# xuelunshen/gim

Hardware: AMD Instinct MI355X
Metric: image-pairs/sec at 640x480 (higher is better)
Workload: dtype fp16

## Files before the change

gim_amd/csrc/bneck_tail.hip:

```cpp
#include "gim_common.h"

namespace {

template <int P, int N1, int NW = 8, bool DS = false> struct Cfg {
    static constexpr int ROWS = 32 * NW;
    static constexpr int LDS_LIMIT = (NW == 8 ? 160 : 80) * 1024;
    static constexpr int C4 = 4 * P;
    static constexpr int KD = DS ? 2 * P : 0;
    static constexpr int CH = (P == 128 && !DS) ? 64 : 32;
    static constexpr int NCHUNK = C4 / CH;
    static constexpr int W3ROW = (P + KD) * 2;
    static constexpr int W3C = CH * W3ROW;
    static constexpr int W1ROW = CH * 2;
    static constexpr int W1C = N1 * W1ROW;
    static constexpr int BUF = W3C + W1C;
    static constexpr int PROW = CH * 2;
    static constexpr int PATCH = 32 * PROW;
    static constexpr int NBUF = (3 * BUF + NW * PATCH + (C4 + N1) * 4 <= LDS_LIMIT) ? 3 : 2;
    static constexpr int OFF_PATCH = NBUF * BUF;
    static constexpr int OFF_BIAS = OFF_PATCH + NW * PATCH;
    static constexpr int SMEM = OFF_BIAS + (C4 + N1) * 4;
    static constexpr int PIECES = BUF / 1024;
    static constexpr int PPW = PIECES / NW;
    static constexpr int IPC = PATCH / 1024;
    static_assert(SMEM <= LDS_LIMIT && PIECES % NW == 0 && (P == 128 || P == 256) && (NW == 8 || NW == 4) && NW * 4096 <= NBUF * BUF && (!DS || P == 128) &&
                  W3C % 1024 == 0, "LDS map");
};

struct Args {
    const unsigned short* t2;
    const unsigned short* res;
    unsigned short* xo;
    unsigned short* t1n;
    const unsigned short* w3;
    const unsigned short* w1n;
    const float* b3;
    const float* b1n;
    int M;
    int act1;
    unsigned w3_bytes, w1n_bytes;
    int* health;
    const unsigned short* xin;
    int Ho, Wo, Hin, Win;
};

typedef __attribute__((address_space(3))) void lds_t;
GIM_TT_DECL(bneck_tail)

typedef gim_u32x4_t u32x4_t;
__device__ __forceinline__ void dma16(const u32x4_t rsrc, unsigned lds_addr, unsigned voff) { gim_dma16(rsrc, lds_addr, voff); }
__device__ __forceinline__ u32x4_t make_rsrc(const void* p, unsigned bytes) { return gim_make_rsrc(p, bytes); }
template <int N> __device__ __forceinline__ void tail_wait() { asm volatile("s_waitcnt vmcnt(%0)" : : "n"(N) : "memory"); }

template <int ROWB> __device__ __forceinline__ int swz(int row, int slot) {
    if constexpr (ROWB >= 256) return (slot & ~15) | ((slot & 15) ^ (row & 15));
    else if constexpr (ROWB == 128) return slot ^ ((row >> 1) & 7);
    else return slot ^ ((row >> 2) & 3);
}
template <int PROW> __device__ __forceinline__ int pswz(int px, int slot) {
    if constexpr (PROW == 128) return slot ^ (px & 7);
    else return slot ^ ((px >> 2) & 3);
}

template <int P, int N1, int NW, bool DS>
__device__ __forceinline__ void issue_chunk(const u32x4_t rw3, const u32x4_t rw1, unsigned smem_addr, int buf, int q, int w, int lane) {
    typedef Cfg<P, N1, NW, DS> C;
    constexpr int S3 = C::W3ROW / 16, S1 = C::W1ROW / 16;
    const unsigned base = smem_addr + (unsigned)(buf * C::BUF);
#pragma unroll
    for (int k = 0; k < C::PPW; ++k) {
        const int pc = w + NW * k;
        if (pc < C::W3C / 1024) {
            const int idx = pc * 64 + lane, n = idx / S3, d = idx % S3;
            const unsigned voff = (unsigned)((q * C::CH + n) * C::W3ROW + (swz<C::W3ROW>(n, d) << 4));
            dma16(rw3, base + (unsigned)(pc * 1024), voff);
        } else {
            const int p1 = pc - C::W3C / 1024;
            const int idx = p1 * 64 + lane, n = idx / S1, d = idx % S1;
            const unsigned voff = (unsigned)((q * N1 + n) * C::W1ROW + (swz<C::W1ROW>(n, d) << 4));
            dma16(rw1, base + (unsigned)(C::W3C + p1 * 1024), voff);
        }
    }
}

template <int P, int N1, int NW, bool DS = false>
__global__ void __launch_bounds__(NW * 64, 2) bneck_tail_kernel(const Args a) {
    typedef Cfg<P, N1, NW, DS> C;
    constexpr int ROWS = C::ROWS;
    constexpr int C4 = C::C4, CH = C::CH, NCHUNK = C::NCHUNK, PROW = C::PROW;
    constexpr int NF = N1 / 32;
    constexpr int TF = CH / 32;
    constexpr int LPP = PROW / 16;
    constexpr int PPI = 64 / LPP;
    extern __shared__ __attribute__((aligned(16))) char smem[];
    const int lane = threadIdx.x & 63, l31 = lane & 31, lh = lane >> 5;
    const int w = __builtin_amdgcn_readfirstlane(threadIdx.x >> 6);
    bool hbig = false;
    const size_t prow0 = (size_t)blockIdx.x * ROWS + w * 32;
    char* patch = smem + C::OFF_PATCH + w * C::PATCH;

    GIM_TT(bneck_tail, w, 0);
    unsigned long long tt_wait = 0, tt_c3 = 0, tt_epi = 0, tt_c1 = 0, tt_a = 0, tt_b = 0;
    (void)tt_wait; (void)tt_c3; (void)tt_epi; (void)tt_c1; (void)tt_a; (void)tt_b;
    const u32x4_t rw3 = make_rsrc(a.w3, a.w3_bytes), rw1 = make_rsrc(a.w1n, a.w1n_bytes);
    const unsigned smem_addr = __builtin_amdgcn_readfirstlane((unsigned)(size_t)(lds_t*)smem);
    issue_chunk<P, N1, NW, DS>(rw3, rw1, smem_addr, 0, 0, w, lane);
    float* bias = (float*)(smem + C::OFF_BIAS);
    for (int t = threadIdx.x; t < (C4 + N1) / 4; t += NW * 64) {
        if (t < C4 / 4) *(float4*)(bias + 4 * t) = *(const float4*)(a.b3 + 4 * t);
        else *(float4*)(bias + 4 * t) = *(const float4*)(a.b1n + 4 * t - C4);
    }
    bf16x8_t t2[P / 16];
    {
        const unsigned short* tp = a.t2 + (prow0 + l31) * P + 8 * lh;
#pragma unroll
        for (int s = 0; s < P / 16; ++s) t2[s] = *(const bf16x8_t*)(tp + 16 * s);
    }
#pragma unroll
    for (int s = 0; s < P / 16; ++s) asm volatile("" : "+v"(t2[s]));
    bf16x8_t xi[DS ? C::KD / 16 : 1];
    if constexpr (DS) {
        const size_t m = prow0 + l31;
        const int ox = (int)(m % (size_t)a.Wo);
        const size_t r_ = m / (size_t)a.Wo;
        const int oy = (int)(r_ % (size_t)a.Ho);
        const size_t ib = r_ / (size_t)a.Ho;
        const unsigned short* xp = a.xin + ((ib * a.Hin + 2 * oy) * a.Win + 2 * ox) * C::KD + 8 * lh;
#pragma unroll
        for (int s = 0; s < C::KD / 16; ++s) xi[s] = *(const bf16x8_t*)(xp + 16 * s);
#pragma unroll
        for (int s = 0; s < C::KD / 16; ++s) asm volatile("" : "+v"(xi[s]));
    }
    const u32x4_t rres = make_rsrc(DS ? (const void*)a.t2 : (const void*)a.res, DS ? 16u : (unsigned)((size_t)a.M * C4 * 2));
    const unsigned patch_addr = smem_addr + (unsigned)(C::OFF_PATCH + w * C::PATCH);
    const int ipx = lane / LPP, isl = lane % LPP;
    const unsigned id_voff = (unsigned)((prow0 + ipx) * (C4 * 2)) + (unsigned)(pswz<PROW>(ipx, isl) << 4);
    auto issue_identity = [&](const int q) __attribute__((always_inline)) {
        if constexpr (!DS) {
#pragma unroll
            for (int k = 0; k < C::IPC; ++k) dma16(rres, patch_addr + (unsigned)(k * 1024), id_voff + (unsigned)(k * PPI * C4 * 2 + q * CH * 2));
        }
    };
    issue_identity(0);
    if constexpr (C::NBUF == 3) issue_chunk<P, N1, NW, DS>(rw3, rw1, smem_addr, 1, 1, w, lane);
    __syncthreads();

    GIM_TT(bneck_tail, w, 1);
    f32x16_t c1[NF];
#pragma unroll
    for (int f = 0; f < NF; ++f) {
#pragma unroll
        for (int rg = 0; rg < 4; ++rg) {
            const float4 bb = *(const float4*)(bias + C4 + 32 * f + 8 * rg + 4 * lh);
            c1[f][rg * 4] = bb.x; c1[f][rg * 4 + 1] = bb.y; c1[f][rg * 4 + 2] = bb.z; c1[f][rg * 4 + 3] = bb.w;
        }
    }

#pragma unroll 1
    for (int q = 0; q < NCHUNK; ++q) {
        tt_a = GIM_TT_NOW();
        const bool dma_ahead = C::NBUF == 3 && q + 1 < NCHUNK;
        const bool stores_behind = q > 0 && a.xo != nullptr;
        if (dma_ahead) { if (stores_behind) tail_wait<C::PPW + C::IPC>(); else tail_wait<C::PPW>(); }
        else { if (stores_behind) tail_wait<C::IPC>(); else tail_wait<0>(); }
        __syncthreads();
        const char* wb3 = smem + (q % C::NBUF) * C::BUF;
        const char* wb1 = wb3 + C::W3C;
        tt_b = GIM_TT_NOW(); tt_wait += tt_b - tt_a;

        f32x16_t c3[TF];
#pragma unroll
        for (int f = 0; f < TF; ++f) {
#pragma unroll
            for (int rg = 0; rg < 4; ++rg) {
                const float4 bb = *(const float4*)(bias + q * CH + 32 * f + 8 * rg + 4 * lh);
                c3[f][rg * 4] = bb.x; c3[f][rg * 4 + 1] = bb.y; c3[f][rg * 4 + 2] = bb.z; c3[f][rg * 4 + 3] = bb.w;
            }
        }
#pragma unroll
        for (int s = 0; s < P / 16; ++s) {
#pragma unroll
            for (int f = 0; f < TF; ++f) {
                const int n = 32 * f + l31;
                const bf16x8_t wv = *(const bf16x8_t*)(wb3 + n * C::W3ROW + (swz<C::W3ROW>(n, 2 * s + lh) << 4));
                c3[f] = mfma_h16_32x32x16(wv, t2[s], c3[f]);
            }
        }
        if constexpr (DS) {
#pragma unroll
            for (int s = 0; s < C::KD / 16; ++s) {
#pragma unroll
                for (int f = 0; f < TF; ++f) {
                    const int n = 32 * f + l31;
                    const bf16x8_t wv = *(const bf16x8_t*)(wb3 + n * C::W3ROW + (swz<C::W3ROW>(n, 2 * (P / 16 + s) + lh) << 4));
                    c3[f] = mfma_h16_32x32x16(wv, xi[s], c3[f]);
                }
            }
        }
        tt_a = GIM_TT_NOW(); tt_c3 += tt_a - tt_b;
#pragma unroll
        for (int f = 0; f < TF; ++f) {
#pragma unroll
            for (int rg = 0; rg < 4; ++rg) {
                if constexpr (DS) {
#pragma unroll
                    for (int e = 0; e < 4; ++e) c3[f][rg * 4 + e] = fmaxf(c3[f][rg * 4 + e], 0.f);
                } else {
                    const uint2 r = *(const uint2*)(patch + l31 * PROW + (pswz<PROW>(l31, 4 * f + rg) << 4) + lh * 8);
                    c3[f][rg * 4] = fmaxf(c3[f][rg * 4] + h16_lo(r.x), 0.f);
                    c3[f][rg * 4 + 1] = fmaxf(c3[f][rg * 4 + 1] + h16_hi(r.x), 0.f);
                    c3[f][rg * 4 + 2] = fmaxf(c3[f][rg * 4 + 2] + h16_lo(r.y), 0.f);
                    c3[f][rg * 4 + 3] = fmaxf(c3[f][rg * 4 + 3] + h16_hi(r.y), 0.f);
                }
            }
        }
        asm volatile("s_waitcnt lgkmcnt(0)" ::: "memory");
        bf16x8_t xq[2 * TF];
#pragma unroll
        for (int f = 0; f < TF; ++f) {
            unsigned u[8];
#pragma unroll
            for (int rg = 0; rg < 4; ++rg) {
                u[2 * rg] = cvt_pk_h16(c3[f][rg * 4], c3[f][rg * 4 + 1]);
                u[2 * rg + 1] = cvt_pk_h16(c3[f][rg * 4 + 2], c3[f][rg * 4 + 3]);
                *(uint2*)(patch + l31 * PROW + (pswz<PROW>(l31, 4 * f + rg) << 4) + lh * 8) = make_uint2(u[2 * rg], u[2 * rg + 1]);
            }
            xq[2 * f] = __builtin_bit_cast(bf16x8_t, make_uint4(u[0], u[1], u[2], u[3]));
            xq[2 * f + 1] = __builtin_bit_cast(bf16x8_t, make_uint4(u[4], u[5], u[6], u[7]));
        }
        asm volatile("s_waitcnt lgkmcnt(0)" ::: "memory");
        const char* prd = patch + ipx * PROW + (pswz<PROW>(ipx, isl) << 4);
        uint4 x0 = *(const uint4*)(prd), x1 = *(const uint4*)(prd + PPI * PROW), x2 = x0, x3 = x0;
        if constexpr (C::IPC == 4) { x2 = *(const uint4*)(prd + 2 * PPI * PROW); x3 = *(const uint4*)(prd + 3 * PPI * PROW); }
        asm volatile("s_waitcnt lgkmcnt(0)" ::: "memory");
        h16_range_track(hbig, x0); h16_range_track(hbig, x1);
        if constexpr (C::IPC == 4) { h16_range_track(hbig, x2); h16_range_track(hbig, x3); }
        if (q + 1 < NCHUNK) issue_identity(q + 1);
        if (q + C::NBUF - 1 < NCHUNK) issue_chunk<P, N1, NW, DS>(rw3, rw1, smem_addr, (q + C::NBUF - 1) % C::NBUF, q + C::NBUF - 1, w, lane);
        if (a.xo != nullptr) {
            unsigned short* xp = a.xo + (prow0 + ipx) * C4 + CH * q + isl * 8;
            *(uint4*)(xp) = x0; *(uint4*)(xp + (size_t)PPI * C4) = x1;
            if constexpr (C::IPC == 4) { *(uint4*)(xp + (size_t)2 * PPI * C4) = x2; *(uint4*)(xp + (size_t)3 * PPI * C4) = x3; }
        }
        tt_b = GIM_TT_NOW(); tt_epi += tt_b - tt_a;
#pragma unroll
        for (int s = 0; s < 2 * TF; ++s) {
#pragma unroll
            for (int f = 0; f < NF; ++f) {
                const int n = 32 * f + l31;
                const bf16x8_t wv = *(const bf16x8_t*)(wb1 + n * C::W1ROW + (swz<C::W1ROW>(n, 2 * s + lh) << 4));
                c1[f] = mfma_h16_32x32x16(wv, xq[s], c1[f]);
            }
        }
        tt_a = GIM_TT_NOW(); tt_c1 += tt_a - tt_b;
    }
    GIM_TT(bneck_tail, w, 2);
    GIM_TT_SET(bneck_tail, w, 4, tt_wait); GIM_TT_SET(bneck_tail, w, 5, tt_c3); GIM_TT_SET(bneck_tail, w, 6, tt_epi); GIM_TT_SET(bneck_tail, w, 7, tt_c1);
    __syncthreads();
    char* opatch = smem + w * 4096;
    const bool relu1 = a.act1 == GIM_ACT_RELU;
#pragma unroll
    for (int h2 = 0; h2 < NF / 2; ++h2) {
#pragma unroll
        for (int ff = 0; ff < 2; ++ff)
#pragma unroll
            for (int rg = 0; rg < 4; ++rg) {
                const f32x16_t& c = c1[2 * h2 + ff];
                const float lo = relu1 ? 0.f : -INFINITY;
                *(uint2*)(opatch + l31 * 128 + (((4 * ff + rg) ^ (l31 & 7)) << 4) + lh * 8) =
                    make_uint2(cvt_pk_h16(fmaxf(c[rg * 4], lo), fmaxf(c[rg * 4 + 1], lo)), cvt_pk_h16(fmaxf(c[rg * 4 + 2], lo), fmaxf(c[rg * 4 + 3], lo)));
            }
        asm volatile("s_waitcnt lgkmcnt(0)" ::: "memory");
#pragma unroll
        for (int it = 0; it < 4; ++it) {
            const int px = it * 8 + (lane >> 3), sl = lane & 7;
            const uint4 v = *(const uint4*)(opatch + px * 128 + ((sl ^ (px & 7)) << 4));
            *(uint4*)(a.t1n + (prow0 + px) * N1 + 64 * h2 + sl * 8) = v;
        }
        asm volatile("s_waitcnt lgkmcnt(0)" ::: "memory");
    }
    h16_range_flag(a.health, hbig);
    GIM_TT(bneck_tail, w, 3);
}

template <int P, int N1, int NW = 8, bool DS = false>
int launch_tail(const Args& a, hipStream_t s) {
    typedef Cfg<P, N1, NW, DS> C;
    static GimPerDevice attr;
    if (attr.needed()) {
        hipError_t e = hipFuncSetAttribute((const void*)bneck_tail_kernel<P, N1, NW, DS>, hipFuncAttributeMaxDynamicSharedMemorySize, C::SMEM);
        if (e != hipSuccess) { gim_set_error("bneck_tail: hipFuncSetAttribute(%d B LDS): %s", C::SMEM, hipGetErrorString(e)); return GIM_ERR_LAUNCH; }
        attr.done();
    }
    hipLaunchKernelGGL((bneck_tail_kernel<P, N1, NW, DS>), dim3((unsigned)(a.M / C::ROWS)), dim3(NW * 64), C::SMEM, s, a);
    return gim_check_launch("bneck_tail");
}

int tail_entry(int P, const void* t2, const void* res, void* x_out, void* t1_next, const void* w3, const void* w1n,
               const float* b3, const float* b1n, int M, int n_next, int act_next, int32_t* health, gim_stream_t stream) {
    GIM_REQUIRE(t2 && res && t1_next && w3 && w1n && b3 && b1n, "bneck_tail: NULL pointer");
    GIM_REQUIRE(act_next == GIM_ACT_RELU || act_next == GIM_ACT_NONE, "bneck_tail: activation of the next conv1 must be relu or none");
    GIM_REQUIRE(M > 0 && M % 256 == 0, "bneck_tail: the pixel row count must be a multiple of 256 (got %d)", M);
    GIM_REQUIRE((int64_t)M * 4 * P * 2 < (int64_t)0xFFFFFFF0ll, "bneck_tail: tensor too large for 32-bit buffer offsets");
    Args a;
    a.t2 = (const unsigned short*)t2; a.res = (const unsigned short*)res; a.xo = (unsigned short*)x_out; a.t1n = (unsigned short*)t1_next;
    a.w3 = (const unsigned short*)w3; a.w1n = (const unsigned short*)w1n; a.b3 = b3; a.b1n = b1n; a.M = M; a.act1 = act_next;
    a.w3_bytes = (unsigned)(4 * P * P * 2); a.w1n_bytes = (unsigned)(n_next * 4 * P * 2); a.health = (int*)health;
    a.xin = nullptr; a.Ho = a.Wo = a.Hin = a.Win = 0;
    if (P == 128) {
        GIM_REQUIRE(n_next == 128 || n_next == 256, "bneck_tail128: n_next must be 128 or 256 (got %d)", n_next);
        return n_next == 128 ? launch_tail<128, 128>(a, (hipStream_t)stream) : launch_tail<128, 256>(a, (hipStream_t)stream);
    }
    GIM_REQUIRE(n_next == 256, "bneck_tail256: n_next must be 256 (got %d)", n_next);
    if (M / 256 > 256 && M / 256 < 3 * 256) return launch_tail<256, 256, 4>(a, (hipStream_t)stream);
    return launch_tail<256, 256>(a, (hipStream_t)stream);
}

}

extern "C" int GIM_FN(gim_bneck_tail128)(const void* t2, const void* res, void* x_out, void* t1_next, const void* w3, const void* w1n,
                                         const float* b3, const float* b1n, int M, int n_next, int act_next, int32_t* health, gim_stream_t stream) {
    GIM_REQUIRE(x_out, "bneck_tail128: NULL x_out");
    return tail_entry(128, t2, res, x_out, t1_next, w3, w1n, b3, b1n, M, n_next, act_next, health, stream);
}

extern "C" int GIM_FN(gim_bneck_tail128_ds)(const void* t2, const void* x_in, void* x_out, void* t1_next, const void* w3ds, const void* w1n,
                                            const float* b3ds, const float* b1n, int B, int Ho, int Wo, int Hin, int Win, int n_next, int act_next,
                                            int32_t* health, gim_stream_t stream) {
    GIM_REQUIRE(t2 && x_in && x_out && t1_next && w3ds && w1n && b3ds && b1n, "bneck_tail128_ds: NULL pointer");
    GIM_REQUIRE(act_next == GIM_ACT_RELU || act_next == GIM_ACT_NONE, "bneck_tail128_ds: activation of the next conv1 must be relu or none");
    GIM_REQUIRE(B > 0 && Ho > 0 && Wo > 0 && Hin >= 2 * Ho - 1 && Win >= 2 * Wo - 1, "bneck_tail128_ds: the input map must cover the stride-2 samples (%d x %d -> %d x %d)", Hin, Win, Ho, Wo);
    const int64_t M = (int64_t)B * Ho * Wo;
    GIM_REQUIRE(M % 256 == 0, "bneck_tail128_ds: the pixel row count must be a multiple of 256 (got %lld)", (long long)M);
    GIM_REQUIRE(M * 512 * 2 < (int64_t)0xFFFFFFF0ll, "bneck_tail128_ds: tensor too large for 32-bit buffer offsets");
    GIM_REQUIRE(n_next == 128, "bneck_tail128_ds: n_next must be 128 (got %d)", n_next);
    Args a;
    a.t2 = (const unsigned short*)t2; a.res = nullptr; a.xo = (unsigned short*)x_out; a.t1n = (unsigned short*)t1_next;
    a.w3 = (const unsigned short*)w3ds; a.w1n = (const unsigned short*)w1n; a.b3 = b3ds; a.b1n = b1n; a.M = (int)M; a.act1 = act_next;
    a.w3_bytes = (unsigned)(512 * 384 * 2); a.w1n_bytes = (unsigned)(n_next * 512 * 2); a.health = (int*)health;
    a.xin = (const unsigned short*)x_in; a.Ho = Ho; a.Wo = Wo; a.Hin = Hin; a.Win = Win;
    return launch_tail<128, 128, 8, true>(a, (hipStream_t)stream);
}

extern "C" int GIM_FN(gim_bneck_tail256)(const void* t2, const void* res, void* x_out, void* t1_next, const void* w3, const void* w1n,
                                         const float* b3, const float* b1n, int M, int n_next, int act_next, int32_t* health, gim_stream_t stream) {
    return tail_entry(256, t2, res, x_out, t1_next, w3, w1n, b3, b1n, M, n_next, act_next, health, stream);
}
```

Baseline: 816.5.

## Make bottleneck tail kernel persistent with cross-tile weight and operand prefetch

Turns the bottleneck tail kernel into a persistent kernel. The grid is capped at the CU count (two blocks per CU for 4-wave blocks), and each workgroup walks a contiguous range of row tiles. Weight chunks, identity patches and the next tile's t2/x operands are prefetched across tile boundaries, so the DMA pipeline and global loads stay busy between tiles instead of draining at every block. The x output stores now go through buffer stores, and the t1 output staging reuses a weight buffer. In exchange the wait counting and sync logic get more complex, and there are fewer workgroups to hide latency.

```diff
diff --git a/gim_amd/csrc/bneck_tail.hip b/gim_amd/csrc/bneck_tail.hip
--- a/gim_amd/csrc/bneck_tail.hip
+++ b/gim_amd/csrc/bneck_tail.hip
@@ -23,7 +23,7 @@
     static constexpr int PIECES = BUF / 1024;
     static constexpr int PPW = PIECES / NW;
     static constexpr int IPC = PATCH / 1024;
-    static_assert(SMEM <= LDS_LIMIT && PIECES % NW == 0 && (P == 128 || P == 256) && (NW == 8 || NW == 4) && NW * 4096 <= NBUF * BUF && (!DS || P == 128) &&
+    static_assert(SMEM <= LDS_LIMIT && PIECES % NW == 0 && (P == 128 || P == 256) && (NW == 8 || NW == 4) && NW * 4096 <= BUF && (!DS || P == 128) &&
                   W3C % 1024 == 0, "LDS map");
 };
 
@@ -83,7 +83,17 @@
     }
 }
 
-template <int P, int N1, int NW, bool DS = false>
+template <int A, int B, int T> __device__ __forceinline__ void tail_wait_behind(const bool dma_ahead, const bool stores_behind, const bool t1_behind) {
+    if (dma_ahead) {
+        if (stores_behind) { if (t1_behind) tail_wait<A + B + T>(); else tail_wait<A + B>(); }
+        else { if (t1_behind) tail_wait<A + T>(); else tail_wait<A>(); }
+    } else {
+        if (stores_behind) { if (t1_behind) tail_wait<B + T>(); else tail_wait<B>(); }
+        else { if (t1_behind) tail_wait<T>(); else tail_wait<0>(); }
+    }
+}
+
+template <int P, int N1, int NW = 8, bool DS = false>
 __global__ void __launch_bounds__(NW * 64, 2) bneck_tail_kernel(const Args a) {
     typedef Cfg<P, N1, NW, DS> C;
     constexpr int ROWS = C::ROWS;
@@ -92,17 +102,23 @@
     constexpr int TF = CH / 32;
     constexpr int LPP = PROW / 16;
     constexpr int PPI = 64 / LPP;
+    constexpr int T1S = NF / 2 * 4;
     extern __shared__ __attribute__((aligned(16))) char smem[];
-    const int lane = threadIdx.x & 63, l31 = lane & 31, lh = lane >> 5;
+    const int lane_id = threadIdx.x & 63, lane = lane_id, l31 = lane & 31, lh = lane >> 5;
     const int w = __builtin_amdgcn_readfirstlane(threadIdx.x >> 6);
     bool hbig = false;
-    const size_t prow0 = (size_t)blockIdx.x * ROWS + w * 32;
     char* patch = smem + C::OFF_PATCH + w * C::PATCH;
+    const int ntiles = a.M / ROWS, nwg = (int)gridDim.x, bid = (int)blockIdx.x;
+    const int tq = ntiles / nwg, tr = ntiles % nwg;
+    const int tile0 = bid * tq + (bid < tr ? bid : tr), ntile = tq + (bid < tr ? 1 : 0);
+    const int last_g = ntile * NCHUNK - 1;
+    auto prow_of = [&](const int tile) __attribute__((always_inline)) { return (size_t)tile * ROWS + w * 32; };
 
     GIM_TT(bneck_tail, w, 0);
-    unsigned long long tt_wait = 0, tt_c3 = 0, tt_epi = 0, tt_c1 = 0, tt_a = 0, tt_b = 0;
-    (void)tt_wait; (void)tt_c3; (void)tt_epi; (void)tt_c1; (void)tt_a; (void)tt_b;
+    unsigned long long tt_wait = 0, tt_c3 = 0, tt_epi = 0, tt_c1 = 0, tt_out = 0, tt_a = 0, tt_b = 0;
+    (void)tt_wait; (void)tt_c3; (void)tt_epi; (void)tt_c1; (void)tt_out; (void)tt_a; (void)tt_b;
     const u32x4_t rw3 = make_rsrc(a.w3, a.w3_bytes), rw1 = make_rsrc(a.w1n, a.w1n_bytes);
+    const __amdgpu_buffer_rsrc_t rxo = __builtin_amdgcn_make_buffer_rsrc(a.xo, (short)0, a.xo != nullptr ? (int)((unsigned)a.M * (unsigned)(C4 * 2)) : 0, 0x00020000);
     const unsigned smem_addr = __builtin_amdgcn_readfirstlane((unsigned)(size_t)(lds_t*)smem);
     issue_chunk<P, N1, NW, DS>(rw3, rw1, smem_addr, 0, 0, w, lane);
     float* bias = (float*)(smem + C::OFF_BIAS);
@@ -111,60 +127,62 @@
         else *(float4*)(bias + 4 * t) = *(const float4*)(a.b1n + 4 * t - C4);
     }
     bf16x8_t t2[P / 16];
-    {
-        const unsigned short* tp = a.t2 + (prow0 + l31) * P + 8 * lh;
+    bf16x8_t xi[DS ? C::KD / 16 : 1];
+    auto load_operands = [&](const int tile) __attribute__((always_inline)) {
+        const size_t prow = prow_of(tile);
+        const unsigned short* tp = a.t2 + (prow + l31) * P + 8 * lh;
 #pragma unroll
         for (int s = 0; s < P / 16; ++s) t2[s] = *(const bf16x8_t*)(tp + 16 * s);
-    }
-#pragma unroll
-    for (int s = 0; s < P / 16; ++s) asm volatile("" : "+v"(t2[s]));
-    bf16x8_t xi[DS ? C::KD / 16 : 1];
-    if constexpr (DS) {
-        const size_t m = prow0 + l31;
-        const int ox = (int)(m % (size_t)a.Wo);
-        const size_t r_ = m / (size_t)a.Wo;
-        const int oy = (int)(r_ % (size_t)a.Ho);
-        const size_t ib = r_ / (size_t)a.Ho;
-        const unsigned short* xp = a.xin + ((ib * a.Hin + 2 * oy) * a.Win + 2 * ox) * C::KD + 8 * lh;
-#pragma unroll
-        for (int s = 0; s < C::KD / 16; ++s) xi[s] = *(const bf16x8_t*)(xp + 16 * s);
-#pragma unroll
-        for (int s = 0; s < C::KD / 16; ++s) asm volatile("" : "+v"(xi[s]));
-    }
+        if constexpr (DS) {
+            const size_t m = prow + l31;
+            const int ox = (int)(m % (size_t)a.Wo);
+            const size_t r_ = m / (size_t)a.Wo;
+            const int oy = (int)(r_ % (size_t)a.Ho);
+            const size_t ib = r_ / (size_t)a.Ho;
+            const unsigned short* xp = a.xin + ((ib * a.Hin + 2 * oy) * a.Win + 2 * ox) * C::KD + 8 * lh;
+#pragma unroll
+            for (int s = 0; s < C::KD / 16; ++s) xi[s] = *(const bf16x8_t*)(xp + 16 * s);
+        }
+    };
+    auto fence_operands = [&]() __attribute__((always_inline)) {
+#pragma unroll
+        for (int s = 0; s < P / 16; ++s) asm volatile("" : "+v"(t2[s]));
+        if constexpr (DS) {
+#pragma unroll
+            for (int s = 0; s < C::KD / 16; ++s) asm volatile("" : "+v"(xi[s]));
+        }
+    };
+    load_operands(tile0);
     const u32x4_t rres = make_rsrc(DS ? (const void*)a.t2 : (const void*)a.res, DS ? 16u : (unsigned)((size_t)a.M * C4 * 2));
     const unsigned patch_addr = smem_addr + (unsigned)(C::OFF_PATCH + w * C::PATCH);
     const int ipx = lane / LPP, isl = lane % LPP;
-    const unsigned id_voff = (unsigned)((prow0 + ipx) * (C4 * 2)) + (unsigned)(pswz<PROW>(ipx, isl) << 4);
-    auto issue_identity = [&](const int q) __attribute__((always_inline)) {
+    const unsigned id_key = (unsigned)(ipx * (C4 * 2)) + (unsigned)(pswz<PROW>(ipx, isl) << 4);
+    auto issue_identity = [&](const int tile, const int q) __attribute__((always_inline)) {
         if constexpr (!DS) {
+            const unsigned id_voff = (unsigned)(prow_of(tile) * (C4 * 2)) + id_key;
 #pragma unroll
             for (int k = 0; k < C::IPC; ++k) dma16(rres, patch_addr + (unsigned)(k * 1024), id_voff + (unsigned)(k * PPI * C4 * 2 + q * CH * 2));
         }
     };
-    issue_identity(0);
+    issue_identity(tile0, 0);
     if constexpr (C::NBUF == 3) issue_chunk<P, N1, NW, DS>(rw3, rw1, smem_addr, 1, 1, w, lane);
+    fence_operands();
     __syncthreads();
 
     GIM_TT(bneck_tail, w, 1);
     f32x16_t c1[NF];
-#pragma unroll
-    for (int f = 0; f < NF; ++f) {
-#pragma unroll
-        for (int rg = 0; rg < 4; ++rg) {
-            const float4 bb = *(const float4*)(bias + C4 + 32 * f + 8 * rg + 4 * lh);
-            c1[f][rg * 4] = bb.x; c1[f][rg * 4 + 1] = bb.y; c1[f][rg * 4 + 2] = bb.z; c1[f][rg * 4 + 3] = bb.w;
-        }
-    }
-
-#pragma unroll 1
-    for (int q = 0; q < NCHUNK; ++q) {
+
+    auto chunk = [&](const int it, const int q, auto last_of_tile) __attribute__((always_inline)) {
+        constexpr bool LAST = decltype(last_of_tile)::value;
+        const int tile = tile0 + it, g = it * NCHUNK + q;
+        const size_t prow0 = prow_of(tile);
+        int lane = lane_id;
+        asm volatile("" : "+v"(lane));
+        const int l31 = lane & 31, lh = lane >> 5, ipx = lane / LPP, isl = lane % LPP;
         tt_a = GIM_TT_NOW();
-        const bool dma_ahead = C::NBUF == 3 && q + 1 < NCHUNK;
-        const bool stores_behind = q > 0 && a.xo != nullptr;
-        if (dma_ahead) { if (stores_behind) tail_wait<C::PPW + C::IPC>(); else tail_wait<C::PPW>(); }
-        else { if (stores_behind) tail_wait<C::IPC>(); else tail_wait<0>(); }
+        tail_wait_behind<C::PPW, C::IPC, T1S>(C::NBUF == 3 && g + 1 <= last_g, g > 0, !LAST && q == 0 && g > 0);
         __syncthreads();
-        const char* wb3 = smem + (q % C::NBUF) * C::BUF;
+        const char* wb3 = smem + (g % C::NBUF) * C::BUF;
         const char* wb1 = wb3 + C::W3C;
         tt_b = GIM_TT_NOW(); tt_wait += tt_b - tt_a;
 
@@ -196,6 +214,10 @@
                     c3[f] = mfma_h16_32x32x16(wv, xi[s], c3[f]);
                 }
             }
+        }
+        if constexpr (LAST) {
+            __builtin_amdgcn_sched_barrier(0);
+            if (it + 1 < ntile) load_operands(tile + 1);
         }
         tt_a = GIM_TT_NOW(); tt_c3 += tt_a - tt_b;
 #pragma unroll
@@ -235,12 +257,18 @@
         asm volatile("s_waitcnt lgkmcnt(0)" ::: "memory");
         h16_range_track(hbig, x0); h16_range_track(hbig, x1);
         if constexpr (C::IPC == 4) { h16_range_track(hbig, x2); h16_range_track(hbig, x3); }
-        if (q + 1 < NCHUNK) issue_identity(q + 1);
-        if (q + C::NBUF - 1 < NCHUNK) issue_chunk<P, N1, NW, DS>(rw3, rw1, smem_addr, (q + C::NBUF - 1) % C::NBUF, q + C::NBUF - 1, w, lane);
-        if (a.xo != nullptr) {
-            unsigned short* xp = a.xo + (prow0 + ipx) * C4 + CH * q + isl * 8;
-            *(uint4*)(xp) = x0; *(uint4*)(xp + (size_t)PPI * C4) = x1;
-            if constexpr (C::IPC == 4) { *(uint4*)(xp + (size_t)2 * PPI * C4) = x2; *(uint4*)(xp + (size_t)3 * PPI * C4) = x3; }
+        if (g + 1 <= last_g) { if constexpr (LAST) issue_identity(tile + 1, 0); else issue_identity(tile, q + 1); }
+        if (g + C::NBUF - 1 <= last_g) {
+            const int gn = g + C::NBUF - 1;
+            issue_chunk<P, N1, NW, DS>(rw3, rw1, smem_addr, gn % C::NBUF, gn % NCHUNK, w, lane);
+        }
+        {
+            const unsigned xv = (unsigned)(((prow0 + ipx) * C4 + CH * q + isl * 8) * 2);
+            auto st = [&](const uint4 v, const int k) __attribute__((always_inline)) {
+                __builtin_amdgcn_raw_buffer_store_b128(u32x4_t{v.x, v.y, v.z, v.w}, rxo, (int)(xv + (unsigned)(k * PPI * C4 * 2)), 0, 0);
+            };
+            st(x0, 0); st(x1, 1);
+            if constexpr (C::IPC == 4) { st(x2, 2); st(x3, 3); }
         }
         tt_b = GIM_TT_NOW(); tt_epi += tt_b - tt_a;
 #pragma unroll
@@ -253,34 +281,64 @@
             }
         }
         tt_a = GIM_TT_NOW(); tt_c1 += tt_a - tt_b;
-    }
-    GIM_TT(bneck_tail, w, 2);
+    };
+
+#pragma unroll 1
+    for (int it = 0; it < ntile; ++it) {
+#pragma unroll
+        for (int f = 0; f < NF; ++f) {
+#pragma unroll
+            for (int rg = 0; rg < 4; ++rg) {
+                const float4 bb = *(const float4*)(bias + C4 + 32 * f + 8 * rg + 4 * lh);
+                c1[f][rg * 4] = bb.x; c1[f][rg * 4 + 1] = bb.y; c1[f][rg * 4 + 2] = bb.z; c1[f][rg * 4 + 3] = bb.w;
+            }
+        }
+#pragma unroll 1
+        for (int q = 0; q < NCHUNK - 1; ++q) chunk(it, q, std::false_type());
+        chunk(it, NCHUNK - 1, std::true_type());
+        if (it + 1 == ntile) GIM_TT(bneck_tail, w, 2);
+        __syncthreads();
+        const size_t prow0 = prow_of(tile0 + it);
+        char* opatch = smem + ((it * NCHUNK + NCHUNK - 1) % C::NBUF) * C::BUF + w * 4096;
+        const bool relu1 = a.act1 == GIM_ACT_RELU;
+#pragma unroll
+        for (int h2 = 0; h2 < NF / 2; ++h2) {
+#pragma unroll
+            for (int ff = 0; ff < 2; ++ff)
+#pragma unroll
+                for (int rg = 0; rg < 4; ++rg) {
+                    const f32x16_t& c = c1[2 * h2 + ff];
+                    const float lo = relu1 ? 0.f : -INFINITY;
+                    *(uint2*)(opatch + l31 * 128 + (((4 * ff + rg) ^ (l31 & 7)) << 4) + lh * 8) =
+                        make_uint2(cvt_pk_h16(fmaxf(c[rg * 4], lo), fmaxf(c[rg * 4 + 1], lo)), cvt_pk_h16(fmaxf(c[rg * 4 + 2], lo), fmaxf(c[rg * 4 + 3], lo)));
+                }
+            asm volatile("s_waitcnt lgkmcnt(0)" ::: "memory");
+#pragma unroll
+            for (int k = 0; k < 4; ++k) {
+                const int px = k * 8 + (lane >> 3), sl = lane & 7;
+                const uint4 v = *(const uint4*)(opatch + px * 128 + ((sl ^ (px & 7)) << 4));
+                *(uint4*)(a.t1n + (prow0 + px) * N1 + 64 * h2 + sl * 8) = v;
+            }
+            asm volatile("s_waitcnt lgkmcnt(0)" ::: "memory");
+        }
+        fence_operands();
+        tt_b = GIM_TT_NOW(); tt_out += tt_b - tt_a;
+    }
     GIM_TT_SET(bneck_tail, w, 4, tt_wait); GIM_TT_SET(bneck_tail, w, 5, tt_c3); GIM_TT_SET(bneck_tail, w, 6, tt_epi); GIM_TT_SET(bneck_tail, w, 7, tt_c1);
-    __syncthreads();
-    char* opatch = smem + w * 4096;
-    const bool relu1 = a.act1 == GIM_ACT_RELU;
-#pragma unroll
-    for (int h2 = 0; h2 < NF / 2; ++h2) {
-#pragma unroll
-        for (int ff = 0; ff < 2; ++ff)
-#pragma unroll
-            for (int rg = 0; rg < 4; ++rg) {
-                const f32x16_t& c = c1[2 * h2 + ff];
-                const float lo = relu1 ? 0.f : -INFINITY;
-                *(uint2*)(opatch + l31 * 128 + (((4 * ff + rg) ^ (l31 & 7)) << 4) + lh * 8) =
-                    make_uint2(cvt_pk_h16(fmaxf(c[rg * 4], lo), fmaxf(c[rg * 4 + 1], lo)), cvt_pk_h16(fmaxf(c[rg * 4 + 2], lo), fmaxf(c[rg * 4 + 3], lo)));
-            }
-        asm volatile("s_waitcnt lgkmcnt(0)" ::: "memory");
-#pragma unroll
-        for (int it = 0; it < 4; ++it) {
-            const int px = it * 8 + (lane >> 3), sl = lane & 7;
-            const uint4 v = *(const uint4*)(opatch + px * 128 + ((sl ^ (px & 7)) << 4));
-            *(uint4*)(a.t1n + (prow0 + px) * N1 + 64 * h2 + sl * 8) = v;
-        }
-        asm volatile("s_waitcnt lgkmcnt(0)" ::: "memory");
-    }
+    GIM_TT_SET(bneck_tail, w, 8, tt_out); GIM_TT_SET(bneck_tail, w, 9, (unsigned long long)ntile);
     h16_range_flag(a.health, hbig);
     GIM_TT(bneck_tail, w, 3);
+}
+
+int tail_cus() {
+    static std::atomic<int> cus[256];
+    const int d = GimPerDevice::dev();
+    int n = cus[d].load(std::memory_order_relaxed);
+    if (n <= 0) {
+        if (hipDeviceGetAttribute(&n, hipDeviceAttributeMultiprocessorCount, d) != hipSuccess || n <= 0) n = 256;
+        cus[d].store(n, std::memory_order_relaxed);
+    }
+    return n;
 }
 
 template <int P, int N1, int NW = 8, bool DS = false>
@@ -292,7 +350,8 @@
         if (e != hipSuccess) { gim_set_error("bneck_tail: hipFuncSetAttribute(%d B LDS): %s", C::SMEM, hipGetErrorString(e)); return GIM_ERR_LAUNCH; }
         attr.done();
     }
-    hipLaunchKernelGGL((bneck_tail_kernel<P, N1, NW, DS>), dim3((unsigned)(a.M / C::ROWS)), dim3(NW * 64), C::SMEM, s, a);
+    const int tiles = a.M / C::ROWS, slots = tail_cus() * (NW == 8 ? 1 : 2);
+    hipLaunchKernelGGL((bneck_tail_kernel<P, N1, NW, DS>), dim3((unsigned)(tiles < slots ? tiles : slots)), dim3(NW * 64), C::SMEM, s, a);
     return gim_check_launch("bneck_tail");
 }
 
```

Result: no change. 819.9, median of 6 (+0.4%).
